# Jordy-VL/multi-modal-early-exit

Hardware: AMD Instinct MI355X
Metric: docs_per_sec (higher is better)
Workload: dtype f32 (operands split into 2 x f16, 3 f16 MFMA terms per MAC, f32 accumulate)

## Files before the change

include/mmee.h:

```cpp
#ifndef MMEE_H
#define MMEE_H

#include <stddef.h>
#include <stdint.h>

#ifdef __cplusplus
extern "C" {
#endif

#define MMEE_ABI_VERSION 3
#define MMEE_MAX_ENCODER_EXITS 64

enum { MMEE_EXIT_VISION_AVG = 0, MMEE_EXIT_TEXT_AVG = 1, MMEE_EXIT_TEXT_VISUAL_CONCAT = 2 };
enum { MMEE_STRATEGY_RAMP = 0, MMEE_STRATEGY_GATE = 1 };
enum { MMEE_CRIT_MAX_CONFIDENCE = 0, MMEE_CRIT_ENTROPY = 1, MMEE_CRIT_PATIENCE = 2 };
enum { MMEE_ARCH_LAYOUTLMV3 = 0, MMEE_ARCH_BEIT = 1 };
enum { MMEE_PREC_F32 = 0, MMEE_PREC_BF16 = 1, MMEE_PREC_F32_SPLIT = 2 };
enum { MMEE_DT_F32 = 0, MMEE_DT_F16 = 1, MMEE_DT_BF16 = 2 };
enum {
    MMEE_FLAG_DENSE_ROWS = 1,
    MMEE_FLAG_NO_EXIT = 2,
    MMEE_FLAG_WHOLE_LAYERS = 4,
    MMEE_FLAG_PROBE_ALWAYS = 8,
    MMEE_FLAG_ONE_TERM = 32,
    MMEE_FLAG_XPROBE = 16
};

typedef struct ee_handle ee_handle;

typedef struct ee_config {
    int32_t abi_version;
    int32_t hidden_size, num_hidden_layers, num_attention_heads, intermediate_size;
    int32_t vocab_size, max_position_embeddings, type_vocab_size, pad_token_id;
    int32_t max_2d_position_embeddings, coordinate_size, shape_size;
    int32_t rel_pos_bins, max_rel_pos, rel_2d_pos_bins, max_rel_2d_pos;
    int32_t input_size, patch_size, num_channels, num_labels;
    float layer_norm_eps;
    int32_t n_embedding_exits;
    int32_t embedding_exits[3];
// ... 104 lines not shown
```

multi-modal-early-exit_amd/capi.py:

```python
from __future__ import annotations

import ctypes as C
import os
from typing import Optional

ABI_VERSION = 3
MAX_ENCODER_EXITS = 64
EXIT_KIND = {"vision_avg": 0, "text_avg": 1, "text_visual_concat": 2}
FLAG_DENSE_ROWS = 1
FLAG_NO_EXIT = 2
FLAG_WHOLE_LAYERS = 4
FLAG_PROBE_ALWAYS = 8
FLAG_XPROBE = 16
FLAG_ONE_TERM = 32
CRIT_MAX_CONFIDENCE, CRIT_ENTROPY, CRIT_PATIENCE = 0, 1, 2
DT_F32, DT_F16, DT_BF16 = 0, 1, 2
CLOCK_STAMP_WORDS = 4096

_LIB_NAME = "libmmee_hip.so"
_LIB_PATH = os.environ.get("MMEE_LIB") or os.path.join(os.path.dirname(os.path.abspath(__file__)), _LIB_NAME)


class MMEEUnavailable(RuntimeError):
    pass


class MMEEError(RuntimeError):
    pass

# ... 107 lines not shown
```

multi-modal-early-exit_amd/csrc/capi.hip:

```cpp
#include <cmath>
#include <cstdarg>
#include <cstdio>
#include <cstring>
#include <string>
#include <vector>

#include "capi_internal.h"

using namespace mmee;
using namespace mmee::capi;

namespace {

std::string g_create_error;

}

namespace mmee {
namespace capi {

int fail(ee_handle* h, const char* fmt, ...) {
    char buf[1024];
    va_list ap;
    va_start(ap, fmt);
// ... 293 lines not shown
    rc |= dev_alloc(h, &h->vis_raw, Bm * NP * H);
    rc |= dev_alloc(h, &h->text_part, Bm * tch * H);
    rc |= dev_alloc(h, &h->vis_part, Bm * vch * H);
    rc |= dev_alloc(h, &h->cat_part, Bm * (tch + vch) * H);
    for (int k = 0; k < 3; ++k) rc |= dev_alloc(h, &h->pooled[k], Bm * H);
    rc |= dev_alloc(h, &h->hid, Bm * H);
    rc |= dev_alloc(h, &h->hid2, Bm * H);
    rc |= dev_alloc(h, &h->head_logits, Bm * 64);
    rc |= dev_alloc(h, &h->pol_logits, Bm * 64);
    rc |= dev_alloc(h, &h->text_dst, Bm * Tm + 1);
    rc |= dev_alloc(h, &h->emb_pos, Bm * Tm + 1);
    rc |= dev_alloc(h, &h->ntext, Bm);
    rc |= dev_alloc(h, &h->row_src, rows);
    rc |= dev_alloc(h, &h->err_flag, 4);
    h->n_queue_heads = 128 * (12 * L + 4 * (E + 1) + 16);
    rc |= dev_alloc(h, &h->queue_heads, (size_t)h->n_queue_heads);
    rc |= dev_alloc(h, &h->meta[0], rows);
    rc |= dev_alloc(h, &h->meta[1], rows);
    const size_t st = (size_t)(E + 2) * (Bm + 1);
    rc |= dev_alloc(h, &h->doc_orig, st);
    rc |= dev_alloc(h, &h->doc_off, st);
    rc |= dev_alloc(h, &h->x_src, st);
    rc |= dev_alloc(h, &h->meta_src, st);
    rc |= dev_alloc(h, &h->counts, (size_t)(E + 2));
    rc |= dev_alloc(h, &h->thr_dev, 256);
    rc |= dev_alloc(h, &h->pat_state, 2 * Bm);
    return rc;
}

int report_missing(ee_handle* h) {
// ... 214 lines not shown
```

multi-modal-early-exit_amd/csrc/capi_forward.hip:

```cpp
#include <cmath>
#include <cstring>
#include <vector>

#include "capi_internal.h"

using namespace mmee;
using namespace mmee::capi;

namespace {

__global__ void zero_words_kernel(int* __restrict__ a, int na, int* __restrict__ b, int nb) {
    for (int i = blockIdx.x * blockDim.x + threadIdx.x; i < na + nb; i += gridDim.x * blockDim.x) {
        if (i < na) a[i] = 0;
        else b[i - na] = 0;
    }
}

__global__ void set_thresholds_kernel(ThrPack p, double* __restrict__ dst) {
    for (int i = threadIdx.x; i < p.n; i += blockDim.x) dst[i] = p.v[i];
}

int forward_pre(ee_handle* h, hipStream_t s) {
    if (!h->fwd_done) HIP_OK(h, hipEventCreateWithFlags(&h->fwd_done, hipEventDisableTiming));
    if (!h->err_host) {
// ... 39 lines not shown
};

struct Forward {
    ee_handle* const h;
    const ForwardArgs a;
    const ee_handle::GraphRec* const cap;
    const ee_config& c = h->cfg;
    float* const hs_out = h->next_hidden_out;
    const float* const embeds_in = h->next_inputs_embeds;
    const float* const head_mask = h->next_head_mask;
    float* const attn_out = h->next_attn_out;
    const hipStream_t s = reinterpret_cast<hipStream_t>(a.stream);
    const bool beit = c.arch == MMEE_ARCH_BEIT, sp = h->split, patience = c.criterion == MMEE_CRIT_PATIENCE;
    const bool no_exit = a.flags & MMEE_FLAG_NO_EXIT, probe_on = !(a.flags & MMEE_FLAG_WHOLE_LAYERS);
    const bool one_term = (a.flags & MMEE_FLAG_ONE_TERM) && sp && !beit;
    const bool use_idx = sp && attn_variant() == 0 && c.rel_pos_bins <= 64 && c.rel_2d_pos_bins <= 64;
    const bool x_split = sp && !beit;
    const int B = a.B, T = beit ? 0 : a.T;
    const int H = c.hidden_size, I = c.intermediate_size, L = c.num_hidden_layers, K = c.num_labels, E = c.n_embedding_exits + c.n_encoder_exits;
    const int G = c.input_size / c.patch_size, NP = G * G, Pv = NP + 1, cus = h->num_cus;
    const size_t sstride = (size_t)c.max_docs + 1;
    int max_len = 0, max_rows = 0;
    int cur = 0, meta_cur = 0, exit_index = 0, next_enc = 0;
    const int* x_phys = nullptr;
    bool use_row_src = false;
    bool cls_ready = false;

    static int attn_variant() { static const int v = mmee::diag_env_int("MMEE_ATTN_V", 0); return v; }

    Forward(ee_handle* h_, const ForwardArgs& a_, const ee_handle::GraphRec* cap_) : h(h_), a(a_), cap(cap_) {
        h->next_hidden_out = nullptr;
        h->next_inputs_embeds = nullptr;
        h->next_head_mask = nullptr;
        h->next_attn_out = nullptr;
    }

    int* S_doc_orig(int st) const { return h->doc_orig + st * sstride; }
    int* S_doc_off(int st) const { return h->doc_off + st * sstride; }
    int* S_x_src(int st) const { return h->x_src + st * sstride; }
    int* S_meta_src(int st) const { return h->meta_src + st * sstride; }

// ... 17 lines not shown
        if (hs_out && (a.flags & (MMEE_FLAG_NO_EXIT | MMEE_FLAG_WHOLE_LAYERS)) != (MMEE_FLAG_NO_EXIT | MMEE_FLAG_WHOLE_LAYERS))
            return fail(h, "ee_forward: hidden states are collected in dump-all mode with whole layers only (MMEE_FLAG_NO_EXIT | MMEE_FLAG_WHOLE_LAYERS)");
        if (cap && (hs_out || embeds_in || head_mask || attn_out || h->prof_on))
            return fail(h, "ee_graph_capture: the one-shot side inputs / outputs (inputs_embeds, hidden states, head mask, attention maps) and ee_profile "
                           "belong to eager calls");
        return 0;
    }

    int* next_head() {
        if (h->next_queue_head + 128 > h->n_queue_heads) return nullptr;
        int* p = h->queue_heads + h->next_queue_head;
        h->next_queue_head += 128;
        return p;
    }

    GemmArgs gemm_args() const {
        GemmArgs g{};
        g.scale = 1.f; g.prio_mode = 1; g.err_flag = h->err_flag;
        return g;
    }

    void run_gemm(GemmArgs g, int epi) {
        g.terms = one_term ? 1 : 3;
        if (sp) launch_gemm_split(g, epi, max_rows, cus, s);
        else launch_gemm_f32(g, epi, AMODE_ROWS, max_rows, cus, s);
    }

    GemmArgs q_gemm(const LayerW& w, bool split) const {
        GemmArgs g = gemm_args();
        g.W = split ? w.qkv_s : w.qkv_w; g.bias = w.qkv_b; g.N = H; g.K = H; g.alpha = w.qkv_inv / mmee::kSplitScaleX; g.scale_cols = H; g.scale = 0.125f;
        return g;
    }
    GemmArgs qkv_gemm(const LayerW& w, bool split) const {
        GemmArgs g = q_gemm(w, split);
        g.N = 3 * H; g.out_split = split ? 1 : 0; g.out_scale = mmee::kSplitScaleQKV;
        return g;
    }
    GemmArgs attn_out_gemm(const LayerW& w, bool split) const {
        GemmArgs g = gemm_args();
        g.W = split ? w.ao_s : w.ao_w; g.bias = w.ao_b; g.N = H; g.K = H; g.alpha = w.ao_inv / mmee::kSplitScaleCtx; g.col_scale = w.lam1;
// ... 182 lines not shown
        const LayerW& w = h->layers[l];
        const int* rp = &h->counts[cur].n_rows;
        AttnArgs at = attn_args();
        at.qkv_doc_off = qkv_off;
        { ProfScope ps(h, P_ATTN, s); run_attn(at); }
        if (attn_out)
            mmee::launch_attention_probs(h->QKV, 3 * H, sp ? 1 : 0, mmee::kSplitScaleQKV, h->meta[meta_cur], S_doc_off(cur), h->t1, h->tx, h->ty, h->n1, h->c1,
                                         h->n2, h->c2, H, c.num_attention_heads, max_len, B, head_mask ? head_mask + (size_t)l * c.num_attention_heads : nullptr,
                                         attn_out + (size_t)l * B * c.num_attention_heads * max_len * max_len, s);
        if (head_mask)
            mmee::launch_head_scale_ctx(h->CTX, H, rp, max_rows, H, head_mask + (size_t)l * c.num_attention_heads, sp ? 1 : 0, mmee::kSplitScaleCtx, cus,
                                        h->err_flag, s);
        GemmArgs g = attn_out_gemm(w, sp);
        g.A = h->CTX; g.lda = H; g.C = h->Y; g.ldc = H; g.resid = sp ? h->Xs : h->X; g.ldr = H; g.resid_row_src = x_rows;
        g.resid_split_inv = sp ? 1.0f / mmee::kSplitScaleX : 0.f; g.role_tag = 2; g.m_ptr = rp; g.tile_counter = next_head();
        { ProfScope ps(h, P_GAO, s); run_gemm(g, EPI_RESID); }
        { ProfScope ps(h, P_LN, s); ln_rows(h->Y, nullptr, sp ? nullptr : h->Y, sp ? h->Ys : nullptr, w.ao_g, w.ao_beta, rp, max_rows); }
        g = ffn_up_gemm(w, sp);
        g.A = sp ? h->Ys : h->Y; g.lda = H; g.C = h->H1; g.ldc = I; g.m_ptr = rp; g.tile_counter = next_head();
        { ProfScope ps(h, P_GUP, s); run_gemm(g, EPI_GELU); }
        g = ffn_down_gemm(w, sp);
        g.A = h->H1; g.lda = I; g.C = h->X; g.ldc = H; g.resid = sp ? h->Ys : h->Y; g.ldr = H;
        g.resid_split_inv = sp ? 1.0f / mmee::kSplitScaleX : 0.f; g.role_tag = 3; g.m_ptr = rp; g.tile_counter = next_head();
        { ProfScope ps(h, P_GDOWN, s); run_gemm(g, EPI_RESID); }
        { ProfScope ps(h, P_LN, s); ln_rows(h->X, nullptr, sp ? nullptr : h->X, sp ? h->Xs : nullptr, w.f_g, w.f_beta, rp, max_rows); }
        h->rec.layer_stage[l] = cur;
    }

    void layer_probe(int l, bool fin, bool xspace) {
        const LayerW& w = h->layers[l];
        ProfScope ps(h, P_PROBE, s);
        const int* nd = &h->counts[cur].n_docs;
        if (xspace) {
            GemmArgs gq = q_gemm(w, true);
            gq.A = h->Xs; gq.lda = H; gq.row_src = x_phys; gq.C = h->Qc; gq.ldc = H; gq.m_ptr = nd; gq.probe = 1;
            launch_gemm_split(gq, EPI_BIAS, B, cus, s);
            mmee::XProbeArgs xa{};
            xa.xs = reinterpret_cast<const char*>(h->Xs); xa.xs_inv = 1.0f / mmee::kSplitScaleX; xa.x_phys = x_phys; xa.doc_off = S_doc_off(cur);
            xa.doc_orig = S_doc_orig(cur); xa.counts = &h->counts[cur]; xa.qc = h->Qc;
            xa.wk = w.qkv_w + (size_t)H * H; xa.bk = w.qkv_b + H; xa.wv_s = w.qkv_s + (size_t)2 * H * H; xa.wv_inv = w.qkv_inv; xa.bv = w.qkv_b + 2 * H;
// ... 210 lines not shown
        else embed_layoutlmv3();

        ForwardRecord& r = h->rec;
        r.layer_stage.assign(L, -1);
        r.layer_qkv_stage.assign(L, -1);
        r.layer_probe_stage.assign(L, -1);
        r.layer_xprobe.assign(L, 0);
        r.exit_stage.assign(E + 1, 0);
        x_phys = S_x_src(0);
        for (int i = 0; i < c.n_embedding_exits; ++i) {
            const int kind = c.embedding_exits[i];
            run_exit(&h->emb_heads[kind], h->pooled[kind], H, S_doc_orig(cur), false);
        }
        gather_hidden(0, x_out(), x_phys, x_inv());
        dump_hidden(0);
        for (int l = 0; l < L; ++l) layer(l);
        final_exit();
        r.last_B = B; r.last_T = T; r.last_stages = E + 1; r.last_flags = a.flags;
        r.last_gate_heads = a.out_head_logits || a.out_head_crit;
        if (!cap) { const int rc_post = forward_post(h, s); if (rc_post) return rc_post; }
        return launch_status(h, cap ? "ee_graph_capture" : "ee_forward");
    }
};

}

extern "C" {

int ee_forward(ee_handle* h, const int64_t* input_ids, const int64_t* attention_mask, const int64_t* bbox,
               const float* pixel_values, const int64_t* token_type_ids, const int64_t* position_ids, int32_t B, int32_t T,
               const double* thresholds, const double* temperatures, uint32_t flags, float* out_logits, int32_t* out_exit,
// ... 84 lines not shown
```

multi-modal-early-exit_amd/csrc/capi_query.hip:

```cpp
#include <cstring>
#include <vector>

#include "capi_internal.h"

using namespace mmee;
using namespace mmee::capi;

namespace {

const char* const kProfNames[] = {
    "prep|doc_prep_kernel+doc_scan_kernel+row_meta_kernel",
    "embed_text|embed_text_kernel",
    "gemm_patch|patch_split_kernel+gemm_split_kernel<.., 0, false> (f32: gemm_f32_kernel<0,1>)",
    "embed_visual|embed_visual_kernel+pool_finish_kernel",
    "gemm_qkv|gemm_f32_kernel<0,0>",
    "attention|attention_f32_kernel",
    "gemm_attn_out|gemm_f32_kernel<2,0>",
    "layernorm|ln_rows_kernel",
    "gemm_ffn_up|gemm_f32_kernel<1,0>",
    "gemm_ffn_down|gemm_f32_kernel<2,0>",
    "exit_head|gemm_f32_kernel<3,0>+head_out_kernel",
    "exit_decide|exit_decide_kernel (patience: exit_decide_patience_kernel)",
    "compact|compact_rows_kernel",
    "gather_cls|gather_cls_kernel",
    "cls_probe|attention_idx_kernel+gemm_split_kernel<.., 1>+ln_rows_kernel+gather_cls_kernel (CLS rows of an exit layer, before its decision)",
    "pair_index|pair_index_kernel [inside prep]",
    "patch_split|patch_split_kernel [inside gemm_patch]",
    "head_out|head_out_kernel [inside exit_head]",
};

int read_stage_counts(ee_handle* h, void* stream, int n, std::vector<StageCounts>& sc) {
    HIP_OK(h, hipStreamSynchronize(reinterpret_cast<hipStream_t>(stream)));
    sc.resize(n);
// ... 191 lines not shown
```

multi-modal-early-exit_amd/csrc/gemm_split.hip:

```cpp
#include <cstdlib>
#include "mmee_common.h"

#include "gemm_split_kernel.h"

namespace mmee {

bool gemm_split_supports(int N, int K) { return N > 0 && K > 0 && N % 256 == 0 && K % 32 == 0; }

void launch_split_ffn_up(const GemmArgs& a, int max_m, int num_cus, hipStream_t s);

void launch_gemm_split(const GemmArgs& a_in, int epi, int max_m, int num_cus, hipStream_t s) {
    GemmArgs a = a_in;
    a.tile_order = a.N <= 768 ? 1 : 0;
    if (a.probe) a.terms = 3;
    if (a.probe) {
        if (a.out_split && epi == EPI_GELU) { launch_split_one<CfgP, EPI_GELU, true, false, 1>(a, max_m, num_cus, s); return; }
        if (!a.out_split && epi == EPI_RESID) { launch_split_one<CfgP, EPI_RESID, false, false, 1>(a, max_m, num_cus, s); return; }
        if (!a.out_split && epi == EPI_BIAS) { launch_split_one<CfgP, EPI_BIAS, false, false, 1>(a, max_m, num_cus, s); return; }
        if (!a.out_split && epi == EPI_TANH) { launch_split_one<CfgP, EPI_TANH, false, false, 1>(a, max_m, num_cus, s); return; }
    }
    a.k_splits = 1;
    if (a.terms != 1 && (long)((max_m + 255) / 256) * (a.N / 256) * 2 <= (long)num_cus) {
        a.tile_counter = nullptr;
        if (a.out_split && epi == EPI_GELU) { launch_split_one<CfgP, EPI_GELU, true, false, 1>(a, max_m, num_cus, s); return; }
        if (a.out_split && epi == EPI_BIAS) { launch_split_one<CfgP, EPI_BIAS, true, false, 1>(a, max_m, num_cus, s); return; }
        if (!a.out_split && epi == EPI_RESID) { launch_split_one<CfgP, EPI_RESID, false, false, 1>(a, max_m, num_cus, s); return; }
        if (!a.out_split && epi == EPI_BIAS) { launch_split_one<CfgP, EPI_BIAS, false, false, 1>(a, max_m, num_cus, s); return; }
        if (!a.out_split && epi == EPI_TANH) { launch_split_one<CfgP, EPI_TANH, false, false, 1>(a, max_m, num_cus, s); return; }
        a.tile_counter = a_in.tile_counter;
    }
#ifdef MMEE_DIAG
    static const int order_env = diag_env_int("MMEE_GEMM_ORDER", -1);
    if (order_env == 0 || order_env == 1) a.tile_order = order_env;
    else if (order_env == 2) a.tile_order = a.N <= 768 ? 1 : 0;
    else if (order_env == 3 || order_env == 4) a.tile_order = a.N >= 2304 ? order_env - 1 : a.tile_order;
    static const int forced = diag_env_int("MMEE_SPLIT_CFG", 0);
    const bool use_a = forced == 1;
    if (a.dbg_noload && (forced == 0 || forced == 3)) {
        if (a.out_split && epi == EPI_GELU) launch_split_one<CfgC, EPI_GELU, true, true>(a, max_m, num_cus, s);
        else if (a.out_split) launch_split_one<CfgC, EPI_BIAS, true, true>(a, max_m, num_cus, s);
        else launch_split_one<CfgC, EPI_RESID, false, true>(a, max_m, num_cus, s);
        return;
    }
    if (a.dbg_noload) {
        if (a.out_split) launch_split_one<CfgA, EPI_GELU, true, true>(a, max_m, num_cus, s);
        else if (use_a) launch_split_one<CfgA, EPI_RESID, false, true>(a, max_m, num_cus, s);
        else launch_split_one<CfgB, EPI_RESID, false, true>(a, max_m, num_cus, s);
        return;
    }
    if (forced == 1 || forced == 2) {
        if (a.out_split) {
            if (epi == EPI_GELU && use_a) launch_split_one<CfgA, EPI_GELU, true>(a, max_m, num_cus, s);
            else if (epi == EPI_GELU) launch_split_one<CfgB, EPI_GELU, true>(a, max_m, num_cus, s);
            else if (use_a) launch_split_one<CfgA, EPI_BIAS, true>(a, max_m, num_cus, s);
            else launch_split_one<CfgB, EPI_BIAS, true>(a, max_m, num_cus, s);
            return;
        }
        if (use_a) {
            switch (epi) {
                case EPI_BIAS: launch_split_one<CfgA, EPI_BIAS, false>(a, max_m, num_cus, s); break;
                case EPI_GELU: launch_split_one<CfgA, EPI_GELU, false>(a, max_m, num_cus, s); break;
                case EPI_RESID: launch_split_one<CfgA, EPI_RESID, false>(a, max_m, num_cus, s); break;
                default: launch_split_one<CfgA, EPI_TANH, false>(a, max_m, num_cus, s); break;
            }
            return;
        }
        switch (epi) {
            case EPI_BIAS: launch_split_one<CfgB, EPI_BIAS, false>(a, max_m, num_cus, s); break;
            case EPI_GELU: launch_split_one<CfgB, EPI_GELU, false>(a, max_m, num_cus, s); break;
            case EPI_RESID: launch_split_one<CfgB, EPI_RESID, false>(a, max_m, num_cus, s); break;
            default: launch_split_one<CfgB, EPI_TANH, false>(a, max_m, num_cus, s); break;
        }
        return;
    }
#endif
    if (a.terms == 1) {
        if (a.out_split && epi == EPI_GELU) { launch_split_one<CfgC, EPI_GELU, true, false, 0, 1>(a, max_m, num_cus, s); return; }
        if (a.out_split && epi == EPI_BIAS) { launch_split_one<CfgC, EPI_BIAS, true, false, 0, 1>(a, max_m, num_cus, s); return; }
        if (!a.out_split && epi == EPI_RESID) {
            if (a.role_tag == 3) launch_split_one<CfgC, EPI_RESID, false, false, 3, 1>(a, max_m, num_cus, s);
            else launch_split_one<CfgC, EPI_RESID, false, false, 2, 1>(a, max_m, num_cus, s);
            return;
        }
    }
    if (a.out_split) {
        if (epi == EPI_GELU) launch_split_ffn_up(a, max_m, num_cus, s);
        else launch_split_one<CfgC, EPI_BIAS, true>(a, max_m, num_cus, s);
        return;
    }
    switch (epi) {
        case EPI_BIAS: launch_split_one<CfgC, EPI_BIAS, false>(a, max_m, num_cus, s); break;
        case EPI_GELU: launch_split_one<CfgC, EPI_GELU, false>(a, max_m, num_cus, s); break;
        case EPI_RESID:
            if (a.role_tag == 2) launch_split_one<CfgC, EPI_RESID, false, false, 2>(a, max_m, num_cus, s);
            else if (a.role_tag == 3) launch_split_one<CfgC, EPI_RESID, false, false, 3>(a, max_m, num_cus, s);
            else launch_split_one<CfgC, EPI_RESID, false>(a, max_m, num_cus, s);
            break;
        default: launch_split_one<CfgC, EPI_TANH, false>(a, max_m, num_cus, s); break;
    }
}

__global__ __launch_bounds__(256) void split_rows_kernel(const float* __restrict__ src, char* __restrict__ dst, const int* __restrict__ n_rows_ptr,
                                                         int n_rows_static, int K, float scale, int* __restrict__ err_flag) {
    const int n_rows = n_rows_ptr ? *n_rows_ptr : n_rows_static;
    const int k4 = K / 4;
    const size_t total = (size_t)n_rows * k4;
    float amax = 0.f;
    for (size_t i = (size_t)blockIdx.x * 256 + threadIdx.x; i < total; i += (size_t)gridDim.x * 256) {
        const size_t r = i / k4;
        const int c = (int)(i - r * k4) * 4;
        const f32x4 v = *reinterpret_cast<const f32x4*>(src + r * K + c);
        store_split4(dst + r * (size_t)K * 4, c, v, scale, amax);
    }
    split_flag_overflow(amax, err_flag);
// ... 55 lines not shown
```

multi-modal-early-exit_amd/csrc/gemm_split_kernel.h:

```cpp
#pragma once
#include <cstdlib>
#include "mmee_common.h"

namespace mmee {


template <int BM_, int BN_, int ROWB_, int NST_, int WM_, int WN_, int WGS_, int MF_ = 32>
struct SplitCfg {
    static constexpr int BM = BM_, BN = BN_, ROWB = ROWB_, NST = NST_, WM = WM_, WN = WN_, WGS = WGS_;
    static constexpr int MF = MF_;
    static_assert(MF == 32 || (MF == 16 && ROWB == 128), "the 16x16x32 MFMA consumes one 128-byte row (k = 32) per step");
    static constexpr int NW = WM * WN, THREADS = NW * 64;
    static constexpr int KSTAGE = ROWB / 4;
    static constexpr int PROWS = 1024 / ROWB;
    static constexpr int PA = BM / PROWS / NW, PW = BN / PROWS / NW;
    static constexpr int PP = PA + PW;
    static constexpr int A_BYTES = BM * ROWB, STAGE_BYTES = (BM + BN) * ROWB, LOOP_BYTES = NST * STAGE_BYTES;
    static constexpr int EPI_BYTES = NW * 32 * 64 * 4;
    static_assert(BM == WM * 64 && BN == WN * 64, "one 64x64 sub-tile per wave");
    static_assert(PA * PROWS * NW == BM && PW * PROWS * NW == BN && PA >= 1 && PW >= 1, "DMA pieces must tile the stage");
    static_assert(EPI_BYTES <= LOOP_BYTES, "epilogue staging must fit in the stage ring");
    static_assert(NST >= 2 && NST <= 4, "ring depth");
    static_assert(THREADS <= 1024, "a workgroup is at most 16 waves");
    static_assert(WGS * (LOOP_BYTES + 16) <= 160 * 1024, "LDS budget of a CU (160 KiB) for WGS workgroups");
// ... 1 lines not shown
};
using CfgA = SplitCfg<128, 256, 64, 3, 2, 4, 2>;
using CfgB = SplitCfg<256, 256, 128, 2, 4, 4, 1>;
using CfgC = SplitCfg<256, 256, 128, 2, 4, 4, 1, 16>;
using CfgP = SplitCfg<128, 128, 128, 3, 2, 2, 1, 16>;


__device__ __forceinline__ void dma_piece(unsigned voff, unsigned long long base, unsigned lds_addr) {
    unsigned keep;
    asm volatile("s_mov_b32 %0, m0\n\ts_mov_b32 m0, %2\n\ts_nop 0\n\tglobal_load_lds_dwordx4 %1, %3\n\ts_mov_b32 m0, %0"
                 : "=&s"(keep)
                 : "v"(voff), "s"(lds_addr), "s"(base)
                 : "memory");
}

template <int EPI, bool OUT_SPLIT, int WN>
__device__ __forceinline__ void split_store_tile(const GemmArgs& g, float* smem, f32x16 (&acc)[2][2], int m0, int n0, int M,
                                                 int wave, int lane) {
    const int wr = wave / WN, wc = wave % WN;
    const int l31 = lane & 31, hh = lane >> 5;
    float* stg = smem + wave * (32 * 64);
    const int c4 = (lane & 15) * 4;
    const int col = n0 + wc * 64 + c4;
    f32x4 bv = f32x4{0.f, 0.f, 0.f, 0.f};
    if (g.bias) bv = *reinterpret_cast<const f32x4*>(g.bias + col);
    const float sc = (col < g.scale_cols) ? g.scale : 1.0f;
    f32x4 lam = f32x4{1.f, 1.f, 1.f, 1.f};
    if (g.col_scale) lam = *reinterpret_cast<const f32x4*>(g.col_scale + col);
    const float alpha = g.alpha;
    float amax = 0.f;
// ... 100 lines not shown
        for (int j = 0; j < RB / 4; ++j) {
            const int rl = (lane >> 4) + 4 * j;
            const int row = rbase + 4 * j;
            f32x4 v = *reinterpret_cast<const f32x4*>(stg + rl * 64 + (c4 ^ (16 * ((rl >> 2) & 1))));
#pragma unroll
            for (int t = 0; t < 4; t += 2) {
                f32x2 x = __builtin_elementwise_fma(f32x2{v[t], v[t + 1]}, (f32x2)(alpha_e), f32x2{be[t], be[t + 1]});
                if (need_post) x = x * (f32x2)(post);
                if (EPI == EPI_GELU) x = gelu_scaled2(x, gelu_c0, gelu_hs);
                if (EPI == EPI_TANH) { x[0] = tanhf(x[0]) * s_out; x[1] = tanhf(x[1]) * s_out; }
                if (need_lam) x = x * f32x2{lam[t], lam[t + 1]};
                v[t] = x[0];
                v[t + 1] = x[1];
            }
            if (row < M) {
                if (EPI == EPI_RESID) {
                    const int rs = g.resid_row_src ? g.resid_row_src[row] : row;
                    if (g.resid_split_inv != 0.f) {
                        const f32x4 r = load_split4_sum(g.resid + (size_t)rs * g.ldr, col);
#pragma unroll
                        for (int t = 0; t < 4; t += 2) {
                            const f32x2 y = __builtin_elementwise_fma(f32x2{r[t], r[t + 1]}, (f32x2)(g.resid_split_inv), f32x2{v[t], v[t + 1]});
                            v[t] = y[0];
                            v[t + 1] = y[1];
                        }
                    } else {
                        v += *reinterpret_cast<const f32x4*>(g.resid + (size_t)rs * g.ldr + col);
                    }
                }
                if (!OUT_SPLIT) *reinterpret_cast<f32x4*>(g.C + c_shift + (size_t)row * g.ldc + col) = v;
            }
            if (OUT_SPLIT) {
                int2 h2, l2;
                {
                    unsigned h01, h23, l01, l23;
                    split_pair(v[0], v[1], h01, l01, amax);
                    split_pair(v[2], v[3], h23, l23, amax);
                    h2.x = (int)h01; h2.y = (int)h23; l2.x = (int)l01; l2.y = (int)l23;
                }
                const bool take_lo = (lane & 2) != 0;
                int4 piece;
                {
                    const int a0 = __builtin_amdgcn_mov_dpp(h2.x, 0x88, 0xf, 0xf, true), a1 = __builtin_amdgcn_mov_dpp(h2.y, 0x88, 0xf, 0xf, true);
                    const int b0 = __builtin_amdgcn_mov_dpp(l2.x, 0x88, 0xf, 0xf, true), b1 = __builtin_amdgcn_mov_dpp(l2.y, 0x88, 0xf, 0xf, true);
                    const int c0 = __builtin_amdgcn_mov_dpp(h2.x, 0xDD, 0xf, 0xf, true), c1 = __builtin_amdgcn_mov_dpp(h2.y, 0xDD, 0xf, 0xf, true);
// ... 275 lines not shown
            if (have) setup(tm, tn, nxt);
        }
        const int last_slot = (buf0 + nk - 1) % NST;
        const int nbuf0 = HANDOVER ? (last_slot ^ 1) : 0;
        if (HANDOVER && have) issue(nxt, 0, nbuf0);
        if (!(dbg & 8)) {
            if constexpr (Cfg::MF == 16) {
                if constexpr (HANDOVER)
                    split_store_tile16<EPI, OUT_SPLIT, WN, 16>(g, smem + last_slot * (STAGE_BYTES / 4), acc16, m0, n0, M, wave, lane, bv, lam);
                else
                    split_store_tile16<EPI, OUT_SPLIT, WN, 32>(g, smem, acc16, m0, n0, M, wave, lane, bv, lam, c_shift);
            } else {
                split_store_tile<EPI, OUT_SPLIT, WN>(g, smem, acc, m0, n0, M, wave, lane);
            }
        }
        __syncthreads();
        if (!have) break;
        cur = nxt;
        buf0 = nbuf0;
        if (!HANDOVER) {
            issue(cur, 0, 0);
            if (NST >= 3 && nk > 1) issue(cur, 1, 1);
            if (NST >= 4 && nk > 2) issue(cur, 2, 2);
        }
    }
    if (DIAG && g.clk_probe && threadIdx.x == 0) {
        g.clk_probe[2 * blockIdx.x] = __builtin_amdgcn_s_memtime() - clk0;
        g.clk_probe[2 * blockIdx.x + 1] = __builtin_amdgcn_s_memrealtime() - rt0;
    }
}
// ... 14 lines not shown
```

multi-modal-early-exit_amd/csrc/mmee_common.h:

```cpp
#pragma once
#include <hip/hip_runtime.h>
#include <stdint.h>

#include <stdio.h>
#include <stdlib.h>
#include <atomic>
#include <mutex>

namespace mmee {

inline int diag_env_int(const char* name, int dflt) {
#ifdef MMEE_DIAG
    const char* e = getenv(name);
    return e ? atoi(e) : dflt;
#else
    (void)name;
    return dflt;
#endif
}

struct LdsOptInError {
    std::mutex mu;
    int code = 0;
    char what[192] = {0};
// ... 243 lines not shown
        "v_fma_mix_f32 %1, %4, 1.0, %6 op_sel:[1,0,1] op_sel_hi:[1,0,1]\n\t"
        "v_fma_mix_f32 %2, %5, 1.0, %7 op_sel:[0,0,0] op_sel_hi:[1,0,1]\n\t"
        "v_fma_mix_f32 %3, %5, 1.0, %7 op_sel:[1,0,1] op_sel_hi:[1,0,1]"
        : "=&v"(r0), "=&v"(r1), "=&v"(r2), "=&v"(r3)
        : "v"(hi[0]), "v"(hi[1]), "v"(lo[0]), "v"(lo[1]));
    return f32x4{r0, r1, r2, r3};
}
__device__ __forceinline__ f32x4 load_split4(const void* row_base, int col, float inv_scale) {
    return load_split4_sum(row_base, col) * inv_scale;
}
constexpr float kSplitScaleX = 16.0f;
constexpr float kSplitScaleCtx = 64.0f;
constexpr float kSplitScaleH1 = 16.0f;
constexpr float kSplitScaleQKV = 16.0f;

enum { EPI_BIAS = 0, EPI_GELU = 1, EPI_RESID = 2, EPI_TANH = 3 };
enum { AMODE_ROWS = 0, AMODE_IM2COL = 1 };

struct GemmArgs {
    const float* A;
    int lda;
    const int* row_src;
    const float* W;
    const float* bias;
    float* C;
    int ldc;
    const float* resid;
    int ldr;
    float resid_split_inv;
    const int* resid_row_src;
    const int* m_ptr;
// ... 7 lines not shown
    const float* pix;
    int C_in, R, P, G;
    float alpha;
    int out_split;
    float out_scale;
    int use_dma;
    int probe;
    int role_tag;
    int tile_order;
    int prio_mode;
    int terms;
    int dbg_noload;
    int* tile_counter;
    unsigned long long* clk_probe;
    int* err_flag;
};

struct AttnArgs {
    const float* qkv;
    int ld;
    float* ctx;
    int ldc;
    const RowMeta* meta;
    const int* doc_off;
    const StageCounts* counts;
    const float* t1;
    const float* tx;
    const float* ty;
    int n1, c1, n2, c2;
    int H, heads, max_len;
// ... 8 lines not shown
    const int* doc_orig;
    const float *w1, *wx, *wy;
    int bins1, bins2;
    float inv_sqrt_d;
    const int* qkv_doc_off;
    int q_limit;
    int terms;
    int idx16;
    const unsigned char* lut1;
    int n_visual;
    const unsigned* keymask;
    const int* doc_flags;
};

void launch_gemm_f32(const GemmArgs& a, int epi, int amode, int max_m, int num_cus, hipStream_t s);
void launch_gemm_split(const GemmArgs& a, int epi, int max_m, int num_cus, hipStream_t s);
bool gemm_split_supports(int N, int K);
void launch_split_rows(const float* src, void* dst, const int* n_rows_ptr, int n_rows_static, int max_rows, int K, float scale,
                       int num_cus, hipStream_t s, int* err_flag = nullptr);
void launch_patch_split(const float* pix, void* dst, int n_docs, int C, int R, int P, float scale, int num_cus, hipStream_t s, int* err_flag);
void launch_absmax(const float* src, size_t n, float* out_dev, hipStream_t s);
void launch_attention_f32(const AttnArgs& a, int max_docs, int num_cus, hipStream_t s);
unsigned long long* attention_pair_stamps();
unsigned long long* attention_idx_stamps();
bool attention_idx_supports(const AttnArgs& a);
bool attention_idx16_fits(int bins1, int bins2, int n1);
void launch_pair_index16(const RowMeta* meta, const int* doc_off, int n_docs, int nb, const unsigned char* lut1, int c1, int n1,
                         const unsigned char* lut2, int c2, int n2, int bins1, unsigned* out16, size_t doc_stride16, unsigned* out_q0,
                         unsigned* keymask, int* doc_flags, int max_len, hipStream_t s);
void launch_attention_idx(const AttnArgs& a, int max_docs, int num_cus, hipStream_t s);
void launch_pair_index(const RowMeta* meta, const int* doc_off, int n_docs, int nb, const unsigned char* lut1, int c1, int n1,
// ... 10 lines not shown
```

multi-modal-early-exit_amd/engine.py:

```python
from __future__ import annotations

import ctypes as C
import json
import os
from dataclasses import dataclass
from typing import Dict, Mapping, Optional, Sequence, Union

import numpy as np

from . import capi
from .config import ModelConfig, check_patience

try:
    import torch
except Exception as _e:
    torch = None
    _torch_err = _e


@dataclass
class EngineOutput:
    logits: "torch.Tensor"
    exit_layer: "torch.Tensor"
    confidence: "torch.Tensor"
# ... 133 lines not shown
                raise ValueError(f"{name} is required")
            return None
        if isinstance(x, np.ndarray):
            x = torch.from_numpy(x)
        if not x.is_cuda or x.device != self.device:
            x = x.to(self.device, non_blocking=True)
        if x.dtype != dtype:
            x = x.to(dtype)
        return x.contiguous()

    def forward(self, input_ids=None, attention_mask=None, bbox=None, pixel_values=None, token_type_ids=None,
                position_ids=None, thresholds: Optional[Union[float, Sequence[float]]] = None,
                temperatures: Optional[Sequence[float]] = None, dump_all: bool = False, dense_rows: bool = False,
                want_all: bool = False, want_head: bool = False, want_hidden_cls: bool = False,
                validate: bool = False, whole_layers: bool = False, probe_always: bool = False, xprobe: Optional[bool] = None,
                one_term: bool = False, inputs_embeds=None, want_hidden_states: bool = False, out=None, head_mask=None,
                want_attentions: bool = False, patience: Optional[int] = None, _capture: bool = False) -> EngineOutput:
        if not self._finalized:
            raise capi.MMEEError("load_weights() has not been called")
        if patience is not None:
            self.set_patience(patience)
        R = self.cfg.input_size
        px = self._dev(pixel_values, torch.float32, "pixel_values")
        emb = None
        if self.beit:
            if inputs_embeds is not None:
                raise ValueError("inputs_embeds: an image-only model has no text embeddings")
            ids = am = bb = tt = ps = None
            B, T = px.shape[0], 0
            if tuple(px.shape) != (B, self.cfg.num_channels, R, R):
                raise ValueError(f"pixel_values must be (B,{self.cfg.num_channels},{R},{R})")
# ... 71 lines not shown
            whole_layers, xprobe = True, False
            L_, nh = self.cfg.num_hidden_layers, self.cfg.num_attention_heads
            if head_mask is not None:
                hm = self._dev(head_mask, torch.float32, "head_mask")
                if hm.dim() == 1:
                    hm = hm.unsqueeze(0).expand(L_, -1)
                if tuple(hm.shape) != (L_, nh):
                    raise ValueError(f"head_mask must be ({nh},) or ({L_}, {nh})")
                hm = hm.contiguous()
            if want_attentions:
                dense_rows = True
                S = T + (self.cfg.input_size // self.cfg.patch_size) ** 2 + 1
                att = torch.empty((L_, B, nh, S, S), dtype=torch.float32, device=dev)
        flags = ((capi.FLAG_NO_EXIT if dump_all else 0) | (capi.FLAG_DENSE_ROWS if dense_rows else 0) |
                 (capi.FLAG_WHOLE_LAYERS if whole_layers else 0) | (capi.FLAG_PROBE_ALWAYS if probe_always else 0) |
                 (capi.FLAG_XPROBE if xprobe else 0) | (capi.FLAG_ONE_TERM if one_term else 0))
        p = lambda t: C.c_void_p(t.data_ptr()) if t is not None else None
        if _capture:
            if emb is not None or hs is not None or hm is not None or att is not None or validate:
                raise ValueError("capture(): inputs_embeds / hidden states / head_mask / attention maps / validate belong to eager calls")
            gid = C.c_int32(-1)
            with torch.cuda.device(dev):
                cur = torch.cuda.current_stream()
                if getattr(self, "_cap_stream", None) is None:
                    self._cap_stream = torch.cuda.Stream(device=dev)
                self._cap_stream.wait_stream(cur)
                rc = self.lib.ee_graph_capture(self._h, p(ids), p(am), p(bb), p(px), p(tt), p(ps), B, T, thr_c, tmp_c, flags,
                                               p(out_logits), p(out_exit), p(out_conf), p(all_logits), p(all_crit),
                                               p(head_logits), p(head_crit), p(hidden), C.c_void_p(self._cap_stream.cuda_stream), C.byref(gid))
                capi.check(rc, self._h, "ee_graph_capture")
                cur.wait_stream(self._cap_stream)
# ... 188 lines not shown
```

Before: 7129.

## Fuse residual LayerNorm into split-precision attn-out and FFN-down GEMMs

Adds an EPI_RESID_LN epilogue in which the split GEMM writes its residual output with write-through stores. It then bumps a per-row-block atomic counter, and the last tile finishing a 256-row block runs the LayerNorm and split-store for those rows. This removes the two separate ln_rows launches per layer and the extra global read of the GEMM output. The cost is a serialized LN tail on one workgroup per row block, extra atomics and fences, and more queue-head memory. A SEPARATE_LN flag keeps the old path.

```diff
diff --git a/include/mmee.h b/include/mmee.h
--- a/include/mmee.h
+++ b/include/mmee.h
@@ -23,6 +23,7 @@
     MMEE_FLAG_WHOLE_LAYERS = 4,
     MMEE_FLAG_PROBE_ALWAYS = 8,
     MMEE_FLAG_ONE_TERM = 32,
+    MMEE_FLAG_SEPARATE_LN = 64,
     MMEE_FLAG_XPROBE = 16
 };
 
diff --git a/multi-modal-early-exit_amd/capi.py b/multi-modal-early-exit_amd/capi.py
--- a/multi-modal-early-exit_amd/capi.py
+++ b/multi-modal-early-exit_amd/capi.py
@@ -13,6 +13,7 @@
 FLAG_PROBE_ALWAYS = 8
 FLAG_XPROBE = 16
 FLAG_ONE_TERM = 32
+FLAG_SEPARATE_LN = 64
 CRIT_MAX_CONFIDENCE, CRIT_ENTROPY, CRIT_PATIENCE = 0, 1, 2
 DT_F32, DT_F16, DT_BF16 = 0, 1, 2
 CLOCK_STAMP_WORDS = 4096
diff --git a/multi-modal-early-exit_amd/csrc/capi.hip b/multi-modal-early-exit_amd/csrc/capi.hip
--- a/multi-modal-early-exit_amd/csrc/capi.hip
+++ b/multi-modal-early-exit_amd/csrc/capi.hip
@@ -331,6 +331,7 @@
     rc |= dev_alloc(h, &h->row_src, rows);
     rc |= dev_alloc(h, &h->err_flag, 4);
     h->n_queue_heads = 128 * (12 * L + 4 * (E + 1) + 16);
+    h->n_queue_heads += 2 * L * (int)(((rows + 255) / 256 + 15) / 16 * 16);
     rc |= dev_alloc(h, &h->queue_heads, (size_t)h->n_queue_heads);
     rc |= dev_alloc(h, &h->meta[0], rows);
     rc |= dev_alloc(h, &h->meta[1], rows);
diff --git a/multi-modal-early-exit_amd/csrc/capi_forward.hip b/multi-modal-early-exit_amd/csrc/capi_forward.hip
--- a/multi-modal-early-exit_amd/csrc/capi_forward.hip
+++ b/multi-modal-early-exit_amd/csrc/capi_forward.hip
@@ -77,6 +77,7 @@
     const bool beit = c.arch == MMEE_ARCH_BEIT, sp = h->split, patience = c.criterion == MMEE_CRIT_PATIENCE;
     const bool no_exit = a.flags & MMEE_FLAG_NO_EXIT, probe_on = !(a.flags & MMEE_FLAG_WHOLE_LAYERS);
     const bool one_term = (a.flags & MMEE_FLAG_ONE_TERM) && sp && !beit;
+    const bool separate_ln = (a.flags & MMEE_FLAG_SEPARATE_LN) != 0;
     const bool use_idx = sp && attn_variant() == 0 && c.rel_pos_bins <= 64 && c.rel_2d_pos_bins <= 64;
     const bool x_split = sp && !beit;
     const int B = a.B, T = beit ? 0 : a.T;
@@ -88,6 +89,7 @@
     const int* x_phys = nullptr;
     bool use_row_src = false;
     bool cls_ready = false;
+    int sched_err = 0;
 
     static int attn_variant() { static const int v = mmee::diag_env_int("MMEE_ATTN_V", 0); return v; }
 
@@ -135,16 +137,33 @@
         return p;
     }
 
+    int* ln_counters() {
+        const int n = ((max_rows + 255) / 256 + 15) / 16 * 16;
+        if (h->next_queue_head + n > h->n_queue_heads) return nullptr;
+        int* p = h->queue_heads + h->next_queue_head;
+        h->next_queue_head += n;
+        return p;
+    }
+
     GemmArgs gemm_args() const {
         GemmArgs g{};
         g.scale = 1.f; g.prio_mode = 1; g.err_flag = h->err_flag;
         return g;
     }
 
-    void run_gemm(GemmArgs g, int epi) {
+    bool run_gemm(GemmArgs g, int epi) {
         g.terms = one_term ? 1 : 3;
-        if (sp) launch_gemm_split(g, epi, max_rows, cus, s);
-        else launch_gemm_f32(g, epi, AMODE_ROWS, max_rows, cus, s);
+        if (sp) return launch_gemm_split(g, epi, max_rows, cus, s);
+        launch_gemm_f32(g, epi, AMODE_ROWS, max_rows, cus, s);
+        return false;
+    }
+
+    void fuse_ln(GemmArgs& g, float* dst, const float* gamma, const float* beta) {
+        if (!sp || separate_ln) return;
+        if (dst == g.A || dst == g.resid) { sched_err = fail(h, "ee_forward: a fused LayerNorm would write planes its own GEMM reads"); return; }
+        g.ln_counter = ln_counters();
+        if (!g.ln_counter) return;
+        g.ln_dst_split = dst; g.ln_gamma = gamma; g.ln_beta = beta; g.ln_eps = c.layer_norm_eps; g.ln_scale = mmee::kSplitScaleX;
     }
 
     GemmArgs q_gemm(const LayerW& w, bool split) const {
@@ -357,16 +376,19 @@
         GemmArgs g = attn_out_gemm(w, sp);
         g.A = h->CTX; g.lda = H; g.C = h->Y; g.ldc = H; g.resid = sp ? h->Xs : h->X; g.ldr = H; g.resid_row_src = x_rows;
         g.resid_split_inv = sp ? 1.0f / mmee::kSplitScaleX : 0.f; g.role_tag = 2; g.m_ptr = rp; g.tile_counter = next_head();
-        { ProfScope ps(h, P_GAO, s); run_gemm(g, EPI_RESID); }
-        { ProfScope ps(h, P_LN, s); ln_rows(h->Y, nullptr, sp ? nullptr : h->Y, sp ? h->Ys : nullptr, w.ao_g, w.ao_beta, rp, max_rows); }
+        fuse_ln(g, h->Ys, w.ao_g, w.ao_beta);
+        bool fused;
+        { ProfScope ps(h, P_GAO, s); fused = run_gemm(g, EPI_RESID); }
+        if (!fused) { ProfScope ps(h, P_LN, s); ln_rows(h->Y, nullptr, sp ? nullptr : h->Y, sp ? h->Ys : nullptr, w.ao_g, w.ao_beta, rp, max_rows); }
         g = ffn_up_gemm(w, sp);
         g.A = sp ? h->Ys : h->Y; g.lda = H; g.C = h->H1; g.ldc = I; g.m_ptr = rp; g.tile_counter = next_head();
         { ProfScope ps(h, P_GUP, s); run_gemm(g, EPI_GELU); }
         g = ffn_down_gemm(w, sp);
         g.A = h->H1; g.lda = I; g.C = h->X; g.ldc = H; g.resid = sp ? h->Ys : h->Y; g.ldr = H;
         g.resid_split_inv = sp ? 1.0f / mmee::kSplitScaleX : 0.f; g.role_tag = 3; g.m_ptr = rp; g.tile_counter = next_head();
-        { ProfScope ps(h, P_GDOWN, s); run_gemm(g, EPI_RESID); }
-        { ProfScope ps(h, P_LN, s); ln_rows(h->X, nullptr, sp ? nullptr : h->X, sp ? h->Xs : nullptr, w.f_g, w.f_beta, rp, max_rows); }
+        fuse_ln(g, h->Xs, w.f_g, w.f_beta);
+        { ProfScope ps(h, P_GDOWN, s); fused = run_gemm(g, EPI_RESID); }
+        if (!fused) { ProfScope ps(h, P_LN, s); ln_rows(h->X, nullptr, sp ? nullptr : h->X, sp ? h->Xs : nullptr, w.f_g, w.f_beta, rp, max_rows); }
         h->rec.layer_stage[l] = cur;
     }
 
@@ -607,7 +629,10 @@
         }
         gather_hidden(0, x_out(), x_phys, x_inv());
         dump_hidden(0);
-        for (int l = 0; l < L; ++l) layer(l);
+        for (int l = 0; l < L; ++l) {
+            layer(l);
+            if (sched_err) return sched_err;
+        }
         final_exit();
         r.last_B = B; r.last_T = T; r.last_stages = E + 1; r.last_flags = a.flags;
         r.last_gate_heads = a.out_head_logits || a.out_head_crit;
diff --git a/multi-modal-early-exit_amd/csrc/capi_query.hip b/multi-modal-early-exit_amd/csrc/capi_query.hip
--- a/multi-modal-early-exit_amd/csrc/capi_query.hip
+++ b/multi-modal-early-exit_amd/csrc/capi_query.hip
@@ -16,7 +16,8 @@
     "gemm_qkv|gemm_f32_kernel<0,0>",
     "attention|attention_f32_kernel",
     "gemm_attn_out|gemm_f32_kernel<2,0>",
-    "layernorm|ln_rows_kernel",
+    "layernorm|ln_rows_kernel (split precision: zero launches when the residual GEMMs normalise their own rows -- gemm_split_kernel<.., 4, false, false, 2 / 3>, "
+    "timed inside gemm_attn_out / gemm_ffn_down; MMEE_FLAG_SEPARATE_LN or 128 x 128 tiles bring the launches back)",
     "gemm_ffn_up|gemm_f32_kernel<1,0>",
     "gemm_ffn_down|gemm_f32_kernel<2,0>",
     "exit_head|gemm_f32_kernel<3,0>+head_out_kernel",
diff --git a/multi-modal-early-exit_amd/csrc/gemm_split.hip b/multi-modal-early-exit_amd/csrc/gemm_split.hip
--- a/multi-modal-early-exit_amd/csrc/gemm_split.hip
+++ b/multi-modal-early-exit_amd/csrc/gemm_split.hip
@@ -9,24 +9,26 @@
 
 void launch_split_ffn_up(const GemmArgs& a, int max_m, int num_cus, hipStream_t s);
 
-void launch_gemm_split(const GemmArgs& a_in, int epi, int max_m, int num_cus, hipStream_t s) {
+bool launch_gemm_split(const GemmArgs& a_in, int epi, int max_m, int num_cus, hipStream_t s) {
     GemmArgs a = a_in;
+    const bool want_ln = a.ln_dst_split && a.ln_counter && epi == EPI_RESID && !a.out_split && !a.probe && (a.role_tag == 2 || a.role_tag == 3) &&
+                         a.N <= 256 * kMaxNV;
     a.tile_order = a.N <= 768 ? 1 : 0;
     if (a.probe) a.terms = 3;
     if (a.probe) {
-        if (a.out_split && epi == EPI_GELU) { launch_split_one<CfgP, EPI_GELU, true, false, 1>(a, max_m, num_cus, s); return; }
-        if (!a.out_split && epi == EPI_RESID) { launch_split_one<CfgP, EPI_RESID, false, false, 1>(a, max_m, num_cus, s); return; }
-        if (!a.out_split && epi == EPI_BIAS) { launch_split_one<CfgP, EPI_BIAS, false, false, 1>(a, max_m, num_cus, s); return; }
-        if (!a.out_split && epi == EPI_TANH) { launch_split_one<CfgP, EPI_TANH, false, false, 1>(a, max_m, num_cus, s); return; }
+        if (a.out_split && epi == EPI_GELU) { launch_split_one<CfgP, EPI_GELU, true, false, 1>(a, max_m, num_cus, s); return false; }
+        if (!a.out_split && epi == EPI_RESID) { launch_split_one<CfgP, EPI_RESID, false, false, 1>(a, max_m, num_cus, s); return false; }
+        if (!a.out_split && epi == EPI_BIAS) { launch_split_one<CfgP, EPI_BIAS, false, false, 1>(a, max_m, num_cus, s); return false; }
+        if (!a.out_split && epi == EPI_TANH) { launch_split_one<CfgP, EPI_TANH, false, false, 1>(a, max_m, num_cus, s); return false; }
     }
     a.k_splits = 1;
     if (a.terms != 1 && (long)((max_m + 255) / 256) * (a.N / 256) * 2 <= (long)num_cus) {
         a.tile_counter = nullptr;
-        if (a.out_split && epi == EPI_GELU) { launch_split_one<CfgP, EPI_GELU, true, false, 1>(a, max_m, num_cus, s); return; }
-        if (a.out_split && epi == EPI_BIAS) { launch_split_one<CfgP, EPI_BIAS, true, false, 1>(a, max_m, num_cus, s); return; }
-        if (!a.out_split && epi == EPI_RESID) { launch_split_one<CfgP, EPI_RESID, false, false, 1>(a, max_m, num_cus, s); return; }
-        if (!a.out_split && epi == EPI_BIAS) { launch_split_one<CfgP, EPI_BIAS, false, false, 1>(a, max_m, num_cus, s); return; }
-        if (!a.out_split && epi == EPI_TANH) { launch_split_one<CfgP, EPI_TANH, false, false, 1>(a, max_m, num_cus, s); return; }
+        if (a.out_split && epi == EPI_GELU) { launch_split_one<CfgP, EPI_GELU, true, false, 1>(a, max_m, num_cus, s); return false; }
+        if (a.out_split && epi == EPI_BIAS) { launch_split_one<CfgP, EPI_BIAS, true, false, 1>(a, max_m, num_cus, s); return false; }
+        if (!a.out_split && epi == EPI_RESID) { launch_split_one<CfgP, EPI_RESID, false, false, 1>(a, max_m, num_cus, s); return false; }
+        if (!a.out_split && epi == EPI_BIAS) { launch_split_one<CfgP, EPI_BIAS, false, false, 1>(a, max_m, num_cus, s); return false; }
+        if (!a.out_split && epi == EPI_TANH) { launch_split_one<CfgP, EPI_TANH, false, false, 1>(a, max_m, num_cus, s); return false; }
         a.tile_counter = a_in.tile_counter;
     }
 #ifdef MMEE_DIAG
@@ -40,13 +42,13 @@
         if (a.out_split && epi == EPI_GELU) launch_split_one<CfgC, EPI_GELU, true, true>(a, max_m, num_cus, s);
         else if (a.out_split) launch_split_one<CfgC, EPI_BIAS, true, true>(a, max_m, num_cus, s);
         else launch_split_one<CfgC, EPI_RESID, false, true>(a, max_m, num_cus, s);
-        return;
+        return false;
     }
     if (a.dbg_noload) {
         if (a.out_split) launch_split_one<CfgA, EPI_GELU, true, true>(a, max_m, num_cus, s);
         else if (use_a) launch_split_one<CfgA, EPI_RESID, false, true>(a, max_m, num_cus, s);
         else launch_split_one<CfgB, EPI_RESID, false, true>(a, max_m, num_cus, s);
-        return;
+        return false;
     }
     if (forced == 1 || forced == 2) {
         if (a.out_split) {
@@ -54,7 +56,7 @@
             else if (epi == EPI_GELU) launch_split_one<CfgB, EPI_GELU, true>(a, max_m, num_cus, s);
             else if (use_a) launch_split_one<CfgA, EPI_BIAS, true>(a, max_m, num_cus, s);
             else launch_split_one<CfgB, EPI_BIAS, true>(a, max_m, num_cus, s);
-            return;
+            return false;
         }
         if (use_a) {
             switch (epi) {
@@ -63,7 +65,7 @@
                 case EPI_RESID: launch_split_one<CfgA, EPI_RESID, false>(a, max_m, num_cus, s); break;
                 default: launch_split_one<CfgA, EPI_TANH, false>(a, max_m, num_cus, s); break;
             }
-            return;
+            return false;
         }
         switch (epi) {
             case EPI_BIAS: launch_split_one<CfgB, EPI_BIAS, false>(a, max_m, num_cus, s); break;
@@ -71,22 +73,32 @@
             case EPI_RESID: launch_split_one<CfgB, EPI_RESID, false>(a, max_m, num_cus, s); break;
             default: launch_split_one<CfgB, EPI_TANH, false>(a, max_m, num_cus, s); break;
         }
-        return;
+        return false;
     }
 #endif
     if (a.terms == 1) {
-        if (a.out_split && epi == EPI_GELU) { launch_split_one<CfgC, EPI_GELU, true, false, 0, 1>(a, max_m, num_cus, s); return; }
-        if (a.out_split && epi == EPI_BIAS) { launch_split_one<CfgC, EPI_BIAS, true, false, 0, 1>(a, max_m, num_cus, s); return; }
+        if (a.out_split && epi == EPI_GELU) { launch_split_one<CfgC, EPI_GELU, true, false, 0, 1>(a, max_m, num_cus, s); return false; }
+        if (a.out_split && epi == EPI_BIAS) { launch_split_one<CfgC, EPI_BIAS, true, false, 0, 1>(a, max_m, num_cus, s); return false; }
+        if (want_ln) {
+            if (a.role_tag == 3) launch_split_one<CfgC, EPI_RESID_LN, false, false, 3, 1>(a, max_m, num_cus, s);
+            else launch_split_one<CfgC, EPI_RESID_LN, false, false, 2, 1>(a, max_m, num_cus, s);
+            return true;
+        }
         if (!a.out_split && epi == EPI_RESID) {
             if (a.role_tag == 3) launch_split_one<CfgC, EPI_RESID, false, false, 3, 1>(a, max_m, num_cus, s);
             else launch_split_one<CfgC, EPI_RESID, false, false, 2, 1>(a, max_m, num_cus, s);
-            return;
+            return false;
         }
+    }
+    if (want_ln) {
+        if (a.role_tag == 3) launch_split_one<CfgC, EPI_RESID_LN, false, false, 3>(a, max_m, num_cus, s);
+        else launch_split_one<CfgC, EPI_RESID_LN, false, false, 2>(a, max_m, num_cus, s);
+        return true;
     }
     if (a.out_split) {
         if (epi == EPI_GELU) launch_split_ffn_up(a, max_m, num_cus, s);
         else launch_split_one<CfgC, EPI_BIAS, true>(a, max_m, num_cus, s);
-        return;
+        return false;
     }
     switch (epi) {
         case EPI_BIAS: launch_split_one<CfgC, EPI_BIAS, false>(a, max_m, num_cus, s); break;
@@ -98,6 +110,7 @@
             break;
         default: launch_split_one<CfgC, EPI_TANH, false>(a, max_m, num_cus, s); break;
     }
+    return false;
 }
 
 __global__ __launch_bounds__(256) void split_rows_kernel(const float* __restrict__ src, char* __restrict__ dst, const int* __restrict__ n_rows_ptr,
diff --git a/multi-modal-early-exit_amd/csrc/gemm_split_kernel.h b/multi-modal-early-exit_amd/csrc/gemm_split_kernel.h
--- a/multi-modal-early-exit_amd/csrc/gemm_split_kernel.h
+++ b/multi-modal-early-exit_amd/csrc/gemm_split_kernel.h
@@ -39,6 +39,48 @@
                  : "memory");
 }
 
+__device__ __forceinline__ void store_f32x4_wt(float* p, const f32x4 v) {
+    asm volatile("global_store_dwordx4 %0, %1, off sc1\n\ts_nop 1" ::"v"(p), "v"(v) : "memory");
+}
+
+struct LnTile {
+    const float* C;
+    int ldc, H;
+    const float *gamma, *beta;
+    float eps, scale;
+    char* dst;
+    int* err_flag;
+};
+template <int NV, int BM, int NW>
+__device__ __forceinline__ void ln_tile_rows(const LnTile& g, int m0, int M, int wave, int lane) {
+    constexpr int RIF = NV <= 2 ? 4 : NV == 3 ? 3 : 2;
+    const int mend = m0 + BM < M ? m0 + BM : M;
+    const int H = g.H;
+    char* dst = g.dst;
+    float amax = 0.f;
+#pragma unroll 1
+    for (int r0 = m0 + wave; r0 < mend; r0 += NW * RIF) {
+        f32x4 x[RIF][NV];
+#pragma unroll
+        for (int j = 0; j < RIF; ++j) {
+            const int row = r0 + NW * j < mend ? r0 + NW * j : r0;
+            const float* p = g.C + (size_t)row * g.ldc + 4 * lane;
+#pragma unroll
+            for (int i = 0; i < NV; ++i) x[j][i] = *reinterpret_cast<const f32x4*>(p + 256 * i);
+        }
+#pragma unroll
+        for (int j = 0; j < RIF; ++j) {
+            const int row = r0 + NW * j;
+            if (row < mend) {
+                wave_layernorm<NV, true>(x[j], H, lane, g.gamma, g.beta, g.eps);
+#pragma unroll
+                for (int i = 0; i < NV; ++i) store_split4_quad(dst + (size_t)row * H * 4, 4 * lane + 256 * i, x[j][i], g.scale, amax, lane);
+            }
+        }
+    }
+    split_flag_overflow(amax, g.err_flag);
+}
+
 template <int EPI, bool OUT_SPLIT, int WN>
 __device__ __forceinline__ void split_store_tile(const GemmArgs& g, float* smem, f32x16 (&acc)[2][2], int m0, int n0, int M,
                                                  int wave, int lane) {
@@ -169,7 +211,7 @@
                 v[t + 1] = x[1];
             }
             if (row < M) {
-                if (EPI == EPI_RESID) {
+                if (EPI == EPI_RESID || EPI == EPI_RESID_LN) {
                     const int rs = g.resid_row_src ? g.resid_row_src[row] : row;
                     if (g.resid_split_inv != 0.f) {
                         const f32x4 r = load_split4_sum(g.resid + (size_t)rs * g.ldr, col);
@@ -183,7 +225,8 @@
                         v += *reinterpret_cast<const f32x4*>(g.resid + (size_t)rs * g.ldr + col);
                     }
                 }
-                if (!OUT_SPLIT) *reinterpret_cast<f32x4*>(g.C + c_shift + (size_t)row * g.ldc + col) = v;
+                if (EPI == EPI_RESID_LN) store_f32x4_wt(g.C + (size_t)row * g.ldc + col, v);
+                else if (!OUT_SPLIT) *reinterpret_cast<f32x4*>(g.C + c_shift + (size_t)row * g.ldc + col) = v;
             }
             if (OUT_SPLIT) {
                 int2 h2, l2;
@@ -489,6 +532,27 @@
                 split_store_tile<EPI, OUT_SPLIT, WN>(g, smem, acc, m0, n0, M, wave, lane);
             }
         }
+        if constexpr (EPI == EPI_RESID_LN) {
+            static_assert(HANDOVER && BM == 256 && !OUT_SPLIT && !KSPLIT, "the fused LayerNorm exists for the 256 x 256 hand-over configuration");
+            asm volatile("s_waitcnt vmcnt(0)" ::: "memory");
+            __syncthreads();
+            if (tid == 0) *q_slot = __hip_atomic_fetch_add(g.ln_counter + m0 / BM, 1, __ATOMIC_RELAXED, __HIP_MEMORY_SCOPE_AGENT);
+            __syncthreads();
+            if (*q_slot == tiles_n - 1) {
+                if (wave == 0) __builtin_amdgcn_fence(__ATOMIC_ACQUIRE, "agent");
+                asm volatile("s_waitcnt vmcnt(0)" ::: "memory");
+                __syncthreads();
+                LnTile t{g.C, g.ldc, g.N, g.ln_gamma, g.ln_beta, g.ln_eps, g.ln_scale, reinterpret_cast<char*>(g.ln_dst_split), g.err_flag};
+                int ln_lane = lane, ln_wave = wave;
+                asm volatile("" : "+v"(ln_lane), "+s"(ln_wave), "+s"(t.C), "+s"(t.ldc), "+s"(t.H), "+s"(t.gamma), "+s"(t.beta), "+s"(t.dst));
+                switch (t.H >> 8) {
+                    case 1: ln_tile_rows<1, BM, Cfg::NW>(t, m0, M, ln_wave, ln_lane); break;
+                    case 2: ln_tile_rows<2, BM, Cfg::NW>(t, m0, M, ln_wave, ln_lane); break;
+                    case 3: ln_tile_rows<3, BM, Cfg::NW>(t, m0, M, ln_wave, ln_lane); break;
+                    default: ln_tile_rows<4, BM, Cfg::NW>(t, m0, M, ln_wave, ln_lane); break;
+                }
+            }
+        }
         __syncthreads();
         if (!have) break;
         cur = nxt;
diff --git a/multi-modal-early-exit_amd/csrc/mmee_common.h b/multi-modal-early-exit_amd/csrc/mmee_common.h
--- a/multi-modal-early-exit_amd/csrc/mmee_common.h
+++ b/multi-modal-early-exit_amd/csrc/mmee_common.h
@@ -281,7 +281,7 @@
 constexpr float kSplitScaleH1 = 16.0f;
 constexpr float kSplitScaleQKV = 16.0f;
 
-enum { EPI_BIAS = 0, EPI_GELU = 1, EPI_RESID = 2, EPI_TANH = 3 };
+enum { EPI_BIAS = 0, EPI_GELU = 1, EPI_RESID = 2, EPI_TANH = 3, EPI_RESID_LN = 4 };
 enum { AMODE_ROWS = 0, AMODE_IM2COL = 1 };
 
 struct GemmArgs {
@@ -319,6 +319,11 @@
     int* tile_counter;
     unsigned long long* clk_probe;
     int* err_flag;
+    const float *ln_gamma, *ln_beta;
+    float ln_eps;
+    float* ln_dst_split;
+    float ln_scale;
+    int* ln_counter;
 };
 
 struct AttnArgs {
@@ -357,7 +362,7 @@
 };
 
 void launch_gemm_f32(const GemmArgs& a, int epi, int amode, int max_m, int num_cus, hipStream_t s);
-void launch_gemm_split(const GemmArgs& a, int epi, int max_m, int num_cus, hipStream_t s);
+bool launch_gemm_split(const GemmArgs& a, int epi, int max_m, int num_cus, hipStream_t s);
 bool gemm_split_supports(int N, int K);
 void launch_split_rows(const float* src, void* dst, const int* n_rows_ptr, int n_rows_static, int max_rows, int K, float scale,
                        int num_cus, hipStream_t s, int* err_flag = nullptr);
diff --git a/multi-modal-early-exit_amd/engine.py b/multi-modal-early-exit_amd/engine.py
--- a/multi-modal-early-exit_amd/engine.py
+++ b/multi-modal-early-exit_amd/engine.py
@@ -171,7 +171,7 @@
                 temperatures: Optional[Sequence[float]] = None, dump_all: bool = False, dense_rows: bool = False,
                 want_all: bool = False, want_head: bool = False, want_hidden_cls: bool = False,
                 validate: bool = False, whole_layers: bool = False, probe_always: bool = False, xprobe: Optional[bool] = None,
-                one_term: bool = False, inputs_embeds=None, want_hidden_states: bool = False, out=None, head_mask=None,
+                one_term: bool = False, separate_ln: bool = False, inputs_embeds=None, want_hidden_states: bool = False, out=None, head_mask=None,
                 want_attentions: bool = False, patience: Optional[int] = None, _capture: bool = False) -> EngineOutput:
         if not self._finalized:
             raise capi.MMEEError("load_weights() has not been called")
@@ -273,7 +273,8 @@
                 att = torch.empty((L_, B, nh, S, S), dtype=torch.float32, device=dev)
         flags = ((capi.FLAG_NO_EXIT if dump_all else 0) | (capi.FLAG_DENSE_ROWS if dense_rows else 0) |
                  (capi.FLAG_WHOLE_LAYERS if whole_layers else 0) | (capi.FLAG_PROBE_ALWAYS if probe_always else 0) |
-                 (capi.FLAG_XPROBE if xprobe else 0) | (capi.FLAG_ONE_TERM if one_term else 0))
+                 (capi.FLAG_XPROBE if xprobe else 0) | (capi.FLAG_ONE_TERM if one_term else 0) |
+                 (capi.FLAG_SEPARATE_LN if separate_ln else 0))
         p = lambda t: C.c_void_p(t.data_ptr()) if t is not None else None
         if _capture:
             if emb is not None or hs is not None or hm is not None or att is not None or validate:
```

Result: no change. 7087 (-0.6%).
